# harveybc/gym-fx

Measured on AMD Instinct MI355X. Metric: env-steps/sec (whole node) PPO EURUSD-1m 4096 vec-envs, higher is better.
Workload: dtype bf16; 1 GPU; model=PPO MLP(256,256) actor-critic bf16 MFMA, global_batch=524288, seq_len=32, parallelism=dp1, n_envs_per_gpu=4096, rollout_steps=128, obs_dim=260, preprocessor=feature_window_preprocessor, reward=pnl_reward, pairs=1

## Files before the change

### gymfx_amd/algo/ppo.py

```python
from __future__ import annotations

import time
from dataclasses import dataclass
from typing import Any, Dict, List

import torch

from ..envs.vec_env import VecFxEnv
from ..models.lstm import ActorCriticLSTM
from ..models.mlp import ActorCriticMLP
from ..ops import api


@dataclass
class PPOConfig:
    rollout_steps: int = 128
    ppo_epochs: int = 4
    minibatches: int = 8
    gamma: float = 0.99
    gae_lambda: float = 0.95
    clip_eps: float = 0.2
    ent_coef: float = 0.01
    vf_coef: float = 0.5
    lr: float = 3e-4
    max_grad_norm: float = 0.5
    seed: int = 0
    hidden: int = 256
    normalize_adv: bool = True
    shuffle_rows: bool = True
    use_graphs: bool = True
    policy: str = "mlp"
    bptt_len: int = 16
    fused_rollout: bool = False
    rollout_streams: int = 1
    fuse_sample: bool = True
    fuse_head: bool = False
    overlap_gather: bool = False
    fused_opt_tail: bool = True

    @classmethod
    def from_config(cls, cfg: Dict[str, Any]) -> "PPOConfig":
        out = cls()
        mapping = {
            "rollout_steps": "rollout_steps",
            "ppo_epochs": "ppo_epochs",
            "minibatches": "minibatches",
            "gamma": "gamma",
            "gae_lambda": "gae_lambda",
            "clip_eps": "clip_eps",
            "ent_coef": "ent_coef",
            "vf_coef": "vf_coef",
            "lr": "learning_rate",
            "max_grad_norm": "max_grad_norm",
            "hidden": "hidden_size",
            "normalize_adv": "normalize_adv",
            "shuffle_rows": "shuffle_rows",
            "use_graphs": "use_graphs",
            "policy": "policy_model",
            "bptt_len": "bptt_len",
            "rollout_streams": "rollout_streams",
            "fused_rollout": "fused_rollout",
            "fuse_sample": "fuse_sample",
            "fuse_head": "fuse_head",
            "overlap_gather": "overlap_gather",
            "fused_opt_tail": "fused_opt_tail",
        }
        from ..config.merger import convert_type

        for attr, key in mapping.items():
            if cfg.get(key) is not None:
                cur = getattr(out, attr)
                val = convert_type(cfg[key]) if isinstance(cur, bool) else cfg[key]
                setattr(out, attr, type(cur)(val))
        if cfg.get("seed") is not None:
            out.seed = int(cfg["seed"])
        return out


class PPOTrainer:
    def __init__(self, env: VecFxEnv, cfg: PPOConfig, *, rank: int = 0,
# ... 114 lines not shown
        import os as _os
        self._fuse_gather = (
            not self.recurrent and self.device.type == "cuda"
            and cfg.shuffle_rows and not self._overlap
            and _os.environ.get("GYMFX_FUSE_GATHER", "0") == "1")
        self._fm = {"seed": self.shuffle_seed, "minibatches": cfg.minibatches,
                    "ctr_off": -1, "step_base": self.step_base,
                    "mb_ctr": self.mb_ctr}

        self._fused_tail = bool(cfg.fused_opt_tail) and (
            not self.recurrent
            or _os.environ.get("GYMFX_LSTM_OPT_TAIL", "0") == "1")
        self.model.fused_tail = self._fused_tail
        self.model.fuse_norm = (self._fused_tail and world_size <= 1
                                and cfg.max_grad_norm > 0)
        self._mb_ticket = (
            torch.zeros((), dtype=torch.int32, device=dev)
            if self._fused_tail
            and _os.environ.get("GYMFX_GATHER_TICKET", "0") == "1" else None)

        self.global_step = 0
        self.update_count = 0
        self.use_graphs = bool(cfg.use_graphs) and self.device.type == "cuda"
        self._split = (self.device.type == "cuda" and cfg.rollout_streams > 1
                       and N % 2 == 0)
        self._fused = (self.device.type == "cuda" and cfg.fused_rollout
                       and not self.recurrent and cfg.hidden == 256)
        self._fuse_sample = (self.device.type == "cuda" and cfg.fuse_sample
                             and getattr(env, "_native", None) is not None
                             and env.params.action_space_mode != "continuous")
# ... 137 lines not shown
    def _fwd_bwd_body(self, slot: int = 0) -> None:
        cfg, model = self.cfg, self.model
        if self.recurrent:
            head = model.bptt_forward(self.obs_mb_seq, self.done_mb,
                                      self.h0_mb, self.c0_mb, self.bptt)
            api.ppo_loss_bwd(
                head, self.act_mb.view(-1), self.logp_mb.view(-1),
                self.adv_mb.view(-1), self.ret_mb.view(-1), self.dhead,
                clip_eps=cfg.clip_eps, ent_coef=cfg.ent_coef,
                vf_coef=cfg.vf_coef, inv_count=1.0 / self.mb_rows,
                losses=self.losses,
            )
            model.bptt_backward(self.obs_mb_seq, self.done_mb, self.dhead,
                                self.bptt)
            return
        if self._fuse_gather:
            head = model.forward(self.obs_flat, self.acts_train,
                                 a_feistel=self._fm)
        else:
            head = model.forward(self.obs_mb_s[slot], self.acts_train)
        api.ppo_loss_bwd(
            head, self.act_mb_s[slot], self.logp_mb_s[slot],
            self.adv_mb_s[slot], self.ret_mb_s[slot],
            self.dhead, clip_eps=cfg.clip_eps, ent_coef=cfg.ent_coef,
            vf_coef=cfg.vf_coef, inv_count=1.0 / self.mb_rows,
            losses=self.losses,
        )
        if self._fuse_gather:
            model.backward(self.obs_flat, self.acts_train, self.dhead,
                           self.scratch, a_feistel=self._fm)
        else:
            model.backward(self.obs_mb_s[slot], self.acts_train, self.dhead,
                           self.scratch)

    def _mb_body(self, slot: int = 0) -> None:
        self._gather_body(slot)
        self._fwd_bwd_body(slot)

    def _mb_body_noshuffle(self, epoch_mb: int) -> None:
        cfg, model = self.cfg, self.model
        M = self.mb_rows
        mb = epoch_mb % cfg.minibatches
        sl = slice(mb * M, (mb + 1) * M)
        self.obs_mb.copy_(self.obs_flat[sl])
        self.act_mb.copy_(self.act_flat[sl])
        self.logp_mb.copy_(self.logp_flat[sl])
        self.adv_mb.copy_(self.adv_flat[sl])
        self.ret_mb.copy_(self.ret_flat[sl])
        head = model.forward(self.obs_mb, self.acts_train)
        api.ppo_loss_bwd(
            head, self.act_mb, self.logp_mb, self.adv_mb, self.ret_mb,
            self.dhead, clip_eps=cfg.clip_eps, ent_coef=cfg.ent_coef,
            vf_coef=cfg.vf_coef, inv_count=1.0 / M, losses=self.losses,
        )
        model.backward(self.obs_mb, self.acts_train, self.dhead, self.scratch)

    def _opt_body(self) -> None:
        self.model.adam(self.cfg.lr, max_grad_norm=self.cfg.max_grad_norm)

    def _snapshot(self) -> Dict[str, Any]:
        m = self.model
        snap = {
            "params": m.params.clone(), "m": m.m.clone(), "v": m.v.clone(),
# ... 63 lines not shown

    def collect_rollout(self) -> None:
        if self.use_graphs and self._graphs_ready:
            self.g_rollout.replay()
        else:
            self._rollout_body()
            self._gae_body()
        self.global_step += self.T

    def compute_advantages(self) -> None:
        pass

    def update(self, with_stats: bool = True) -> Dict[str, float]:
        cfg = self.cfg
        self.losses.zero_()
        self.mb_ctr.zero_()
        graphs = self.use_graphs and self._graphs_ready
        n_mb = cfg.ppo_epochs * cfg.minibatches
        if not cfg.shuffle_rows:
            for i in range(n_mb):
                self._mb_body_noshuffle(i)
                self._allreduce_grads()
                self._opt_body()
            self.update_count += 1
            return self._stats(n_mb) if with_stats else {}
        def gather(slot: int) -> None:
            if graphs:
                self.g_gather[slot].replay()
            else:
                self._gather_body(slot)

        def fwd_bwd(slot: int) -> None:
            if graphs:
                self.g_fwd_bwd[slot].replay()
            else:
                self._fwd_bwd_body(slot)

        def opt() -> None:
            if graphs:
                self.g_opt.replay()
            else:
                self._opt_body()

        if not self._overlap:
            gather(0)
            for i in range(n_mb):
                fwd_bwd(0)
                self._reducer.start(self.model.grads)
                if i + 1 < n_mb:
                    gather(0)
                self._reducer.finish()
                opt()
            self.update_count += 1
            return self._stats(n_mb) if with_stats else {}
        s2 = self._gs
        main = torch.cuda.current_stream()
        ev_fork = torch.cuda.Event()
        ev_g = [torch.cuda.Event(), torch.cuda.Event()]
        gather(0)
        for i in range(n_mb):
            slot = i & 1
            nxt = slot ^ 1
            if i + 1 < n_mb:
                ev_fork.record()
                with torch.cuda.stream(s2):
                    s2.wait_event(ev_fork)
                    gather(nxt)
                    ev_g[nxt].record()
            fwd_bwd(slot)
            self._reducer.start(self.model.grads)
            self._reducer.finish()
            opt()
            if i + 1 < n_mb:
                main.wait_event(ev_g[nxt])
        self.update_count += 1
        return self._stats(n_mb) if with_stats else {}

    def _stats(self, n_mb: int) -> Dict[str, float]:
        lv = (self.losses / n_mb).cpu()
        return {
            "pi_loss": float(lv[0]),
            "v_loss": float(lv[1]),
            "entropy": float(lv[2]),
            "approx_kl": float(lv[3]),
            "clipfrac": float(lv[4]),
        }

    def _allreduce_grads(self) -> None:
        if self.world_size <= 1:
# ... 94 lines not shown
```

### gymfx_amd/config/defaults.py

```python
from __future__ import annotations

DEFAULT_VALUES = {
    "mode": "inference",
    "driver_mode": "buy_hold",
    "steps": 500,

    "data_feed_plugin": "default_data_feed",
    "broker_plugin": "default_broker",
    "strategy_plugin": "default_strategy",
    "preprocessor_plugin": "default_preprocessor",
    "reward_plugin": "pnl_reward",
    "metrics_plugin": "default_metrics",

    "input_data_file": "examples/data/eurusd.csv",
    "date_column": "DATE_TIME",
    "price_column": "CLOSE",
    "instrument": "EUR_USD",
    "timeframe": "M1",
    "headers": True,
    "max_rows": None,

    "window_size": 32,
    "initial_cash": 10000.0,
    "position_size": 1.0,
# ... 35 lines not shown
    "ppo_epochs": 4,
    "minibatches": 8,
    "bptt_len": 16,
    "learning_rate": 3e-4,
    "gamma": 0.99,
    "gae_lambda": 0.95,
    "clip_eps": 0.2,
    "ent_coef": 0.01,
    "vf_coef": 0.5,
    "max_grad_norm": 0.5,
    "train_updates": 10,
    "use_graphs": True,
    "fuse_sample": True,
    "overlap_gather": False,
    "fused_opt_tail": True,
    "checkpoint_file": None,
    "checkpoint_interval": 0,
    "resume": False,
    "trace_file": None,

    "serve_host": "127.0.0.1",
    "serve_port": 8400,

    "optimization_trials": 16,
    "optimization_steps": 256,
    "optimization_refine_trials": 0,
}
```

### gymfx_amd/models/mlp.py

```python
from __future__ import annotations

import math
from dataclasses import dataclass
from typing import Dict, Optional, Tuple

import torch

from ..ops import api


@dataclass
class _ParamSlice:
    name: str
    shape: Tuple[int, ...]
    sl: slice
    is_weight: bool


class ActorCriticMLP:
    def __init__(
        self,
        obs_dim: int,
        n_actions: int = 3,
        hidden: int = 256,
# ... 125 lines not shown

    def forward(self, obs_bf16: torch.Tensor, acts: Dict[str, torch.Tensor],
                a_feistel: "Optional[dict]" = None) -> torch.Tensor:
        api.gemm(obs_bf16, self.wt("W1"), self.f32("b1"), acts["h1"], act=2,
                 trans_b=True, a_perm=a_feistel)
        api.gemm(acts["h1"], self.wt("W2"), self.f32("b2"), acts["h2"], act=2, trans_b=True)
        api.gemm(acts["h2"], self.wt("W3"), self.f32("b3"), acts["head"], act=0, trans_b=True)
        return acts["head"]

    def forward_hidden(self, obs_bf16: torch.Tensor,
                       acts: Dict[str, torch.Tensor]) -> torch.Tensor:
        api.gemm(obs_bf16, self.wt("W1"), self.f32("b1"), acts["h1"], act=2, trans_b=True)
        api.gemm(acts["h1"], self.wt("W2"), self.f32("b2"), acts["h2"], act=2, trans_b=True)
        return acts["h2"]

    def backward(
        self,
        obs_bf16: torch.Tensor,
        acts: Dict[str, torch.Tensor],
        dhead: torch.Tensor,
        scratch: Dict[str, torch.Tensor],
        a_feistel: "Optional[dict]" = None,
    ) -> None:
        M = dhead.shape[0]
        dh2 = scratch["dh2"]
        dh1 = scratch["dh1"]
        red = not self.fused_tail
        dw_p, db_p, slabs = self._wg_workspace("W3", self.hidden, self.head_dim, True)
        api.wgrad(acts["h2"], dhead, self.grad("W3"), self.grad("b3"),
                  workspace=(dw_p, db_p), slabs=slabs, reduce=red)
        api.gemm(dhead, self.w("W3"), None, dh2, Yact=acts["h2"], trans_b=True,
                 act=1, dact_tanh=True)
        dw_p, db_p, slabs = self._wg_workspace("W2", self.hidden, self.hidden, True)
        api.wgrad(acts["h1"], dh2, self.grad("W2"), self.grad("b2"),
                  workspace=(dw_p, db_p), slabs=slabs, reduce=red)
        api.gemm(dh2, self.w("W2"), None, dh1, Yact=acts["h1"], trans_b=True,
                 act=1, dact_tanh=True)
        dw_p, db_p, slabs = self._wg_workspace("W1", self.obs_dim, self.hidden, True)
        api.wgrad(obs_bf16, dh1, self.grad("W1"), self.grad("b1"),
                  workspace=(dw_p, db_p), slabs=slabs, x_perm=a_feistel,
                  reduce=red)
        if self.fused_tail:
            api.grads_finalize(self._finalize_segments(), self.grads,
                               self._clip_part if self.fuse_norm else None)

    def alloc_scratch(self, M: int) -> Dict[str, torch.Tensor]:
        dev = self.device
# ... 49 lines not shown
```

### gymfx_amd/ops/api.py

```python
from __future__ import annotations

from typing import Optional, Sequence, Tuple

import os

import torch

from . import native

_LSTM_FUSED = os.environ.get("GYMFX_LSTM_FUSED", "1") != "0"
_LSTM_BWD_FUSED = os.environ.get("GYMFX_LSTM_BWD_FUSED", "0") == "1"


def _use_native(t: torch.Tensor) -> bool:
    if t.is_cuda:
        native.require()
        return True
    return False



def gemm(
    A: torch.Tensor,
    B: torch.Tensor,
# ... 452 lines not shown
    dlogits = g_lp.unsqueeze(1) * (onehot - pi)
    dlogits = dlogits + ent_coef * pi * (logpi + H.unsqueeze(1))
    v = head[:, A]
    dv = vf_coef * (v - ret)
    d = torch.cat([dlogits, dv.unsqueeze(1)], dim=1) * inv_count
    dhead.copy_(d.to(torch.bfloat16))
    if losses is not None:
        losses[0] += float((-torch.minimum(surr1, surr2)).sum()) * inv_count
        losses[1] += float((0.5 * (v - ret) ** 2).sum()) * inv_count
        losses[2] += float(H.sum()) * inv_count
        losses[3] += float((old_logp - lp).sum()) * inv_count
        clipped = (ratio > 1 + clip_eps) | (ratio < 1 - clip_eps)
        losses[4] += float(clipped.to(torch.float32).sum()) * inv_count


def adv_normalize(adv: torch.Tensor, part: torch.Tensor) -> None:
    if _use_native(adv):
        native.require().adv_normalize(adv, part)
        return
    mean = adv.mean()
    var = (adv * adv).mean() - mean * mean
    adv.sub_(mean).div_(var.clamp(min=0).sqrt() + 1e-8)


def f32_to_bf16(src: torch.Tensor, dst: torch.Tensor) -> None:
    if _use_native(src):
        native.require().f32_to_bf16(src, dst)
        return
    dst.view(-1).copy_(src.reshape(-1).to(torch.bfloat16))

# ... 169 lines not shown
```

### gymfx_amd/ops/csrc/bindings.cpp

```cpp
#include <torch/extension.h>

#include <c10/hip/HIPStream.h>
#include <hip/hip_runtime.h>

#include <unordered_map>
#include <string>
#include <vector>

#include "env_common.h"

namespace gymfx {

void launch_env_step(const EnvPtrs& P, const EnvParamsK& K, int env_lo,
                     int env_cnt, hipStream_t stream);
void launch_build_obs(const EnvPtrs& P, const EnvParamsK& K, int env_lo,
                      int env_cnt, hipStream_t stream);
void launch_env_step_obs(const EnvPtrs& P, const EnvParamsK& K, int env_lo,
                         int env_cnt, hipStream_t stream);
void launch_gemm(const void* A, const void* B, const float* bias, void* C,
                 const void* Yact, int M, int N, int K, bool trans_b, int act,
                 bool dact_tanh, bool add_bias, bool accum, hipStream_t stream,
                 const FeistelMap* fmp = nullptr);
void launch_lstm_cell_fwd(const void* gates_pre, const void* gates_h,
                          const float* c_prev, float* c_new, void* h_new,
// ... 80 lines not shown
                               int row_offset, int greedy, hipStream_t stream);
void launch_increment_i32(int* ctr, int delta, hipStream_t stream);
void launch_mb_gather(const void* obs_src, const int64_t* act_src,
                      const float* logp_src, const float* adv_src,
                      const float* ret_src, void* obs_mb, int64_t* act_mb,
                      float* logp_mb, float* adv_mb, float* ret_mb, int M,
                      int D, uint32_t n, int half, uint64_t seed,
                      int minibatches, const unsigned long long* step_base,
                      unsigned long long* mb_ctr, hipStream_t stream,
                      int skip_obs = 0, unsigned int* ticket = nullptr);
void launch_ppo_loss_bwd(const float* head, const int64_t* actions,
                         const float* old_logp, const float* adv,
                         const float* ret, void* dhead, int M, int n_actions,
                         float clip_eps, float ent_coef, float vf_coef,
                         float inv_count, float* losses, hipStream_t stream);
void launch_adv_normalize(float* adv, int64_t n, float* part, int nparts,
                          hipStream_t stream);
void launch_f32_to_bf16(const float* in, void* out, int64_t n,
                        hipStream_t stream);
void launch_transpose_bf16(const void* src, void* dst, int K, int N,
                           hipStream_t stream);

namespace {

using TensorMap = std::unordered_map<std::string, torch::Tensor>;

template <typename T>
T* ptr(TensorMap& m, const char* key, bool required = true) {
  auto it = m.find(key);
  if (it == m.end() || !it->second.defined()) {
// ... 961 lines not shown
                     torch::Tensor ret, torch::Tensor dhead, double clip_eps,
                     double ent_coef, double vf_coef, double inv_count,
                     c10::optional<torch::Tensor> losses) {
  check_f32(head, "head");
  check_bf16(dhead, "dhead");
  const int M = (int)head.size(0);
  const int n_actions = (int)head.size(1) - 1;
  gymfx::launch_ppo_loss_bwd(
      head.data_ptr<float>(), actions.data_ptr<int64_t>(),
      old_logp.data_ptr<float>(), adv.data_ptr<float>(), ret.data_ptr<float>(),
      dhead.data_ptr(), M, n_actions, (float)clip_eps, (float)ent_coef,
      (float)vf_coef, (float)inv_count,
      losses.has_value() ? losses->data_ptr<float>() : nullptr, cur_stream());
}

void adv_normalize_op(torch::Tensor adv, torch::Tensor part) {
  check_f32(adv, "adv");
  check_f32(part, "part");
  gymfx::launch_adv_normalize(adv.data_ptr<float>(), adv.numel(),
                              part.data_ptr<float>(), (int)(part.numel() / 2),
                              cur_stream());
}

void f32_to_bf16_op(torch::Tensor in, torch::Tensor out) {
  check_f32(in, "in");
  check_bf16(out, "out");
  gymfx::launch_f32_to_bf16(in.data_ptr<float>(), out.data_ptr(), in.numel(),
                            cur_stream());
}

// ... 90 lines not shown
        py::arg("W1t"), py::arg("b1"), py::arg("W2t"), py::arg("b2"),
        py::arg("W3t"), py::arg("b3"), py::arg("actions"), py::arg("logp"),
        py::arg("value"), py::arg("seed"), py::arg("step"),
        py::arg("step_base") = py::none(), py::arg("row_offset") = 0,
        py::arg("greedy") = false);
  m.def("mb_gather", &mb_gather_op, py::arg("obs_src"), py::arg("act_src"),
        py::arg("logp_src"), py::arg("adv_src"), py::arg("ret_src"),
        py::arg("obs_mb"), py::arg("act_mb"), py::arg("logp_mb"),
        py::arg("adv_mb"), py::arg("ret_mb"), py::arg("seed"),
        py::arg("minibatches"), py::arg("step_base"), py::arg("mb_ctr"),
        py::arg("skip_obs") = false, py::arg("ticket") = py::none());
  m.def("ppo_loss_bwd", &ppo_loss_bwd_op, py::arg("head"), py::arg("actions"),
        py::arg("old_logp"), py::arg("adv"), py::arg("ret"), py::arg("dhead"),
        py::arg("clip_eps"), py::arg("ent_coef"), py::arg("vf_coef"),
        py::arg("inv_count"), py::arg("losses") = py::none());
  m.def("adv_normalize", &adv_normalize_op);
  m.def("f32_to_bf16", &f32_to_bf16_op);
  m.def("transpose_bf16", &transpose_bf16_op);
  py::class_<gymfx::GymFxEngine>(m, "GymFxEngine")
      .def(py::init<const py::dict&, const py::dict&, const py::dict&, const py::dict&>())
      .def("step", &gymfx::GymFxEngine::step, py::arg("actions"),
           py::arg("obs_out"), py::arg("reward_out") = py::none(),
           py::arg("terminated_out") = py::none(),
           py::arg("obs_bf16_out") = py::none(), py::arg("env_lo") = 0,
           py::arg("env_hi") = 0, py::arg("head") = py::none(),
           py::arg("logp_out") = py::none(), py::arg("value_out") = py::none(),
           py::arg("step_base") = py::none(), py::arg("sample_seed") = 0,
           py::arg("sample_step") = 0, py::arg("fuse_obs") = false,
           py::arg("h2") = py::none(), py::arg("w3t") = py::none(),
           py::arg("b3") = py::none(), py::arg("rnn_h") = py::none(),
// ... 8 lines not shown
```

### gymfx_amd/ops/csrc/ppo_kernels.hip

```cpp
#include "env_common.h"

#include <hip/hip_bf16.h>

#include <algorithm>

namespace gymfx {

typedef __attribute__((ext_vector_type(8))) __bf16 bf16x8;
typedef __attribute__((ext_vector_type(4))) float f32x4;

GFX_DEV float bf2f(__bf16 v) { return (float)v; }
GFX_DEV __bf16 f2bf(float v) { return (__bf16)v; }

GFX_DEV float fast_tanh(float x) {
  x = fminf(fmaxf(x, -15.f), 15.f);
  const float e = __builtin_amdgcn_exp2f(x * 2.885390081777927f);
  return 1.f - 2.f * __builtin_amdgcn_rcpf(e + 1.f);
}

GFX_DEV uint32_t feistel_encrypt_once(uint32_t x, int half, uint32_t mask,
                                      uint64_t key) {
  uint32_t a = x & mask;
  uint32_t b = x >> half;
  for (int r = 0; r < 4; ++r) {
// ... 883 lines not shown
    a = sample_categorical(row, n_actions, logz, seed, step, mg);
  }
  actions[m] = a;
  logp[m] = row[a] - logz;
  if (value) value[m] = row[n_actions];
  if (entropy) {
    float h = 0.f;
    for (int j = 0; j < n_actions; ++j) {
      const float lp = row[j] - logz;
      h -= fast_exp(lp) * lp;
    }
    entropy[m] = h;
  }
}

__global__ void ppo_loss_bwd_kernel(
    const float* __restrict__ head, const int64_t* __restrict__ actions,
    const float* __restrict__ old_logp, const float* __restrict__ adv,
    const float* __restrict__ ret, __bf16* __restrict__ dhead, int M,
    int n_actions, float clip_eps, float ent_coef, float vf_coef,
    float inv_count, float* __restrict__ losses) {
  const int m = blockIdx.x * blockDim.x + threadIdx.x;
  float l_pi = 0.f, l_v = 0.f, l_ent = 0.f, l_kl = 0.f, l_clip = 0.f;
  if (m < M) {
    const float* row = head + (int64_t)m * (n_actions + 1);
    __bf16* drow = dhead + (int64_t)m * (n_actions + 1);
    float mx = row[0];
    for (int j = 1; j < n_actions; ++j) mx = fmaxf(mx, row[j]);
    float z = 0.f;
    for (int j = 0; j < n_actions; ++j) z += expf(row[j] - mx);
    const float logz = logf(z) + mx;
    const int a = (int)actions[m];
    const float lp = row[a] - logz;
    const float ratio = expf(lp - old_logp[m]);
    const float A = adv[m];
    const bool clipped = (ratio > 1.f + clip_eps) || (ratio < 1.f - clip_eps);
    const float surr1 = ratio * A;
    const float rclip = fminf(fmaxf(ratio, 1.f - clip_eps), 1.f + clip_eps);
    const float surr2 = rclip * A;
    const float g_lp = (surr1 <= surr2) ? (-A * ratio) : 0.f;
    float H = 0.f;
    for (int j = 0; j < n_actions; ++j) {
      const float lpj = row[j] - logz;
      H -= expf(lpj) * lpj;
    }
    for (int j = 0; j < n_actions; ++j) {
      const float pj = expf(row[j] - logz);
      const float onehot = (j == a) ? 1.f : 0.f;
      float d = g_lp * (onehot - pj);
      d += ent_coef * pj * ((row[j] - logz) + H);
      drow[j] = f2bf(d * inv_count);
    }
    const float v = row[n_actions];
    const float dv = vf_coef * (v - ret[m]);
    drow[n_actions] = f2bf(dv * inv_count);

    l_pi = -fminf(surr1, surr2);
    l_v = 0.5f * (v - ret[m]) * (v - ret[m]);
    l_ent = H;
    l_kl = old_logp[m] - lp;
    l_clip = clipped ? 1.f : 0.f;
  }
  __shared__ float red[256];
  float vals[5] = {l_pi, l_v, l_ent, l_kl, l_clip};
  for (int s = 0; s < 5; ++s) {
    red[threadIdx.x] = vals[s];
    __syncthreads();
    for (int w = 128; w > 0; w >>= 1) {
      if (threadIdx.x < w) red[threadIdx.x] += red[threadIdx.x + w];
      __syncthreads();
    }
    if (threadIdx.x == 0 && losses) atomicAdd(&losses[s], red[0] * inv_count);
    __syncthreads();
  }
}

__global__ void adv_norm_stats_kernel(const float* __restrict__ adv, int64_t n,
                                      float* __restrict__ part ) {
  __shared__ float red[512];
  float s = 0.f, ss = 0.f;
  for (int64_t i = (int64_t)blockIdx.x * blockDim.x + threadIdx.x; i < n;
       i += (int64_t)gridDim.x * blockDim.x) {
    s += adv[i];
    ss += adv[i] * adv[i];
  }
  red[threadIdx.x] = s;
  red[256 + threadIdx.x] = ss;
  __syncthreads();
// ... 1015 lines not shown
    if (act == 0) { if (add_bias) GEMM_LAUNCH(false, 0, false, true); else GEMM_LAUNCH(false, 0, false, false); }
    else if (act == 1) { if (add_bias) GEMM_LAUNCH(false, 1, false, true); else GEMM_LAUNCH(false, 1, false, false); }
    else { if (add_bias) GEMM_LAUNCH(false, 2, false, true); else GEMM_LAUNCH(false, 2, false, false); }
  } else if (trans_b && !dact_tanh) {
    if (act == 0) { if (add_bias) GEMM_LAUNCH(true, 0, false, true); else GEMM_LAUNCH(true, 0, false, false); }
    else if (act == 1) { if (add_bias) GEMM_LAUNCH(true, 1, false, true); else GEMM_LAUNCH(true, 1, false, false); }
    else { if (add_bias) GEMM_LAUNCH(true, 2, false, true); else GEMM_LAUNCH(true, 2, false, false); }
  } else if (trans_b && dact_tanh) {
    GEMM_LAUNCH(true, 1, true, false);
  } else {
    GEMM_LAUNCH(false, 1, true, false);
  }
#undef GEMM_LAUNCH
}

void launch_wgrad(const void* X, const void* dY, float* dW_part, float* db_part,
                  float* dW, float* db, int M, int N, int K, int slabs,
                  hipStream_t stream, const FeistelMap* fmp = nullptr,
                  bool reduce = true) {
  const __bf16* x = reinterpret_cast<const __bf16*>(X);
  const __bf16* dy = reinterpret_cast<const __bf16*>(dY);
  static const int big_env = [] {
    const char* e = getenv("GYMFX_WGRAD_BIG");
    return e ? atoi(e) : -1;
  }();
  const bool big = K >= 128 && N >= 128 &&
                   (big_env >= 0
                        ? big_env != 0
                        : (int64_t)ceil_div(K, 128) * ceil_div(N, 128) * slabs >=
                              384);
// ... 41 lines not shown
    else                                                                      \
      hipLaunchKernelGGL((wgrad_partial_kernel<WDB, FK, FN>), grid,           \
                         dim3(256), 0, stream, x, dy, dW_part, db_part, M, N, \
                         K, slabs, 0);                                        \
  } while (0)
    if (db_part) {
      if (big) WG_PART(true, 4, 4);
      else WG_PART(true, 2, 2);
    } else {
      if (big) WG_PART(false, 4, 4);
      else WG_PART(false, 2, 2);
    }
#undef WG_PART
  }
  if (!reduce) return;
  int64_t elems = (int64_t)K * N;
  if (elems <= 4096) {
    hipLaunchKernelGGL(slab_reduce_small_kernel, dim3((int)elems), dim3(256),
                       0, stream, dW_part, dW, elems, slabs);
  } else {
    int blocks = (int)std::min<int64_t>((elems + 1023) / 1024, 1024);
    hipLaunchKernelGGL(slab_reduce_kernel, dim3(blocks), dim3(256), 0, stream,
                       dW_part, dW, elems, slabs);
  }
  if (db_part && db)
    hipLaunchKernelGGL(slab_reduce_small_kernel, dim3(N), dim3(256), 0, stream,
                       db_part, db, (int64_t)N, slabs);
}

void launch_gae(const float* rewards, const float* values, const bool* dones,
// ... 69 lines not shown
                     stream, head, M, n_actions, seed, step, actions, logp,
                     value, entropy, greedy, step_base, row_offset);
}

void launch_ppo_loss_bwd(const float* head, const int64_t* actions,
                         const float* old_logp, const float* adv,
                         const float* ret, void* dhead, int M, int n_actions,
                         float clip_eps, float ent_coef, float vf_coef,
                         float inv_count, float* losses, hipStream_t stream) {
  hipLaunchKernelGGL(ppo_loss_bwd_kernel, dim3(ceil_div(M, 256)), dim3(256), 0,
                     stream, head, actions, old_logp, adv, ret,
                     reinterpret_cast<__bf16*>(dhead), M, n_actions, clip_eps,
                     ent_coef, vf_coef, inv_count, losses);
}

void launch_adv_normalize(float* adv, int64_t n, float* part, int nparts,
                          hipStream_t stream) {
  hipLaunchKernelGGL(adv_norm_stats_kernel, dim3(nparts), dim3(256), 0, stream,
                     adv, n, part);
  int blocks = (int)std::min<int64_t>((n + 255) / 256, 2048);
  hipLaunchKernelGGL(adv_norm_apply_kernel, dim3(blocks), dim3(256), 0, stream,
                     adv, n, part, nparts);
}

void launch_transpose_bf16(const void* src, void* dst, int K, int N,
                           hipStream_t stream) {
  dim3 grid(ceil_div(K, 64), ceil_div(N, 64));
  hipLaunchKernelGGL(transpose_bf16_kernel, grid, dim3(256), 0, stream,
                     reinterpret_cast<const __bf16*>(src),
                     reinterpret_cast<__bf16*>(dst), K, N);
// ... 11 lines not shown
```

Before: 29.17 million env-steps/sec.

## Fuse PPO head GEMM, loss, weight-grad and tanh data-grad into one kernel

Adds a head_loss_bwd HIP kernel that, per row slab, loads h2 into LDS and then does the rest in one launch: the head GEMM, the PPO loss and its gradient, partial W3/b3 gradients and the tanh-masked dh2 via MFMA. The MLP training path now calls forward_hidden plus this fused op, and the rest of backward skips its head part. Loss accumulation is sharded across 64 rows to cut atomic contention, and the shards are folded once per update. The fused path only runs when ceil(M/slabs) <= 128. Otherwise it falls back to the original unfused sequence, so at large minibatch sizes it may never run.

```diff
diff --git a/gymfx_amd/algo/ppo.py b/gymfx_amd/algo/ppo.py
--- a/gymfx_amd/algo/ppo.py
+++ b/gymfx_amd/algo/ppo.py
@@ -37,6 +37,7 @@
     fuse_head: bool = False
     overlap_gather: bool = False
     fused_opt_tail: bool = True
+    fused_head_bwd: bool = True
 
     @classmethod
     def from_config(cls, cfg: Dict[str, Any]) -> "PPOConfig":
@@ -64,6 +65,7 @@
             "fuse_head": "fuse_head",
             "overlap_gather": "overlap_gather",
             "fused_opt_tail": "fused_opt_tail",
+            "fused_head_bwd": "fused_head_bwd",
         }
         from ..config.merger import convert_type
 
@@ -208,6 +210,10 @@
         self.model.fused_tail = self._fused_tail
         self.model.fuse_norm = (self._fused_tail and world_size <= 1
                                 and cfg.max_grad_norm > 0)
+        self._fused_head = bool(cfg.fused_head_bwd) and not self.recurrent
+        self._loss_shards = (
+            torch.zeros(64, 32, dtype=torch.float32, device=dev)
+            if self._fused_head and self.device.type == "cuda" else None)
         self._mb_ticket = (
             torch.zeros((), dtype=torch.int32, device=dev)
             if self._fused_tail
@@ -375,6 +381,18 @@
             model.bptt_backward(self.obs_mb_seq, self.done_mb, self.dhead,
                                 self.bptt)
             return
+        if self._fused_head and not self._fuse_gather:
+            model.forward_hidden(self.obs_mb_s[slot], self.acts_train)
+            model.head_loss_backward(
+                self.acts_train, self.act_mb_s[slot], self.logp_mb_s[slot],
+                self.adv_mb_s[slot], self.ret_mb_s[slot], self.dhead,
+                self.scratch, clip_eps=cfg.clip_eps, ent_coef=cfg.ent_coef,
+                vf_coef=cfg.vf_coef, inv_count=1.0 / self.mb_rows,
+                losses=self._loss_acc(),
+            )
+            model.backward(self.obs_mb_s[slot], self.acts_train, self.dhead,
+                           self.scratch, skip_head=True)
+            return
         if self._fuse_gather:
             head = model.forward(self.obs_flat, self.acts_train,
                                  a_feistel=self._fm)
@@ -394,6 +412,13 @@
             model.backward(self.obs_mb_s[slot], self.acts_train, self.dhead,
                            self.scratch)
 
+    def _loss_acc(self) -> torch.Tensor:
+        return self.losses if self._loss_shards is None else self._loss_shards
+
+    def _fold_losses(self) -> None:
+        if self._loss_shards is not None:
+            self.losses.add_(self._loss_shards[:, :5].sum(dim=0))
+
     def _mb_body(self, slot: int = 0) -> None:
         self._gather_body(slot)
         self._fwd_bwd_body(slot)
@@ -408,6 +433,17 @@
         self.logp_mb.copy_(self.logp_flat[sl])
         self.adv_mb.copy_(self.adv_flat[sl])
         self.ret_mb.copy_(self.ret_flat[sl])
+        if self._fused_head:
+            model.forward_hidden(self.obs_mb, self.acts_train)
+            model.head_loss_backward(
+                self.acts_train, self.act_mb, self.logp_mb, self.adv_mb,
+                self.ret_mb, self.dhead, self.scratch, clip_eps=cfg.clip_eps,
+                ent_coef=cfg.ent_coef, vf_coef=cfg.vf_coef, inv_count=1.0 / M,
+                losses=self._loss_acc(),
+            )
+            model.backward(self.obs_mb, self.acts_train, self.dhead,
+                           self.scratch, skip_head=True)
+            return
         head = model.forward(self.obs_mb, self.acts_train)
         api.ppo_loss_bwd(
             head, self.act_mb, self.logp_mb, self.adv_mb, self.ret_mb,
@@ -501,6 +537,8 @@
     def update(self, with_stats: bool = True) -> Dict[str, float]:
         cfg = self.cfg
         self.losses.zero_()
+        if self._loss_shards is not None:
+            self._loss_shards.zero_()
         self.mb_ctr.zero_()
         graphs = self.use_graphs and self._graphs_ready
         n_mb = cfg.ppo_epochs * cfg.minibatches
@@ -509,6 +547,7 @@
                 self._mb_body_noshuffle(i)
                 self._allreduce_grads()
                 self._opt_body()
+            self._fold_losses()
             self.update_count += 1
             return self._stats(n_mb) if with_stats else {}
         def gather(slot: int) -> None:
@@ -538,6 +577,7 @@
                     gather(0)
                 self._reducer.finish()
                 opt()
+            self._fold_losses()
             self.update_count += 1
             return self._stats(n_mb) if with_stats else {}
         s2 = self._gs
@@ -560,6 +600,7 @@
             opt()
             if i + 1 < n_mb:
                 main.wait_event(ev_g[nxt])
+        self._fold_losses()
         self.update_count += 1
         return self._stats(n_mb) if with_stats else {}
 
diff --git a/gymfx_amd/config/defaults.py b/gymfx_amd/config/defaults.py
--- a/gymfx_amd/config/defaults.py
+++ b/gymfx_amd/config/defaults.py
@@ -73,6 +73,7 @@
     "fuse_sample": True,
     "overlap_gather": False,
     "fused_opt_tail": True,
+    "fused_head_bwd": True,
     "checkpoint_file": None,
     "checkpoint_interval": 0,
     "resume": False,
diff --git a/gymfx_amd/models/mlp.py b/gymfx_amd/models/mlp.py
--- a/gymfx_amd/models/mlp.py
+++ b/gymfx_amd/models/mlp.py
@@ -163,6 +163,31 @@
         api.gemm(acts["h1"], self.wt("W2"), self.f32("b2"), acts["h2"], act=2, trans_b=True)
         return acts["h2"]
 
+    def head_loss_backward(
+        self,
+        acts: Dict[str, torch.Tensor],
+        actions: torch.Tensor,
+        old_logp: torch.Tensor,
+        adv: torch.Tensor,
+        ret: torch.Tensor,
+        dhead: torch.Tensor,
+        scratch: Dict[str, torch.Tensor],
+        *,
+        clip_eps: float,
+        ent_coef: float,
+        vf_coef: float,
+        inv_count: float,
+        losses: Optional[torch.Tensor] = None,
+    ) -> None:
+        dw_p, db_p, slabs = self._wg_workspace("W3", self.hidden, self.head_dim, True)
+        api.head_loss_bwd(
+            acts["h2"], self.wt("W3"), self.w("W3"), self.f32("b3"), actions,
+            old_logp, adv, ret, acts["head"], dhead, scratch["dh2"],
+            self.grad("W3"), self.grad("b3"), workspace=(dw_p, db_p),
+            slabs=slabs, reduce=not self.fused_tail, clip_eps=clip_eps,
+            ent_coef=ent_coef, vf_coef=vf_coef, inv_count=inv_count,
+            losses=losses)
+
     def backward(
         self,
         obs_bf16: torch.Tensor,
@@ -170,16 +195,18 @@
         dhead: torch.Tensor,
         scratch: Dict[str, torch.Tensor],
         a_feistel: "Optional[dict]" = None,
+        skip_head: bool = False,
     ) -> None:
         M = dhead.shape[0]
         dh2 = scratch["dh2"]
         dh1 = scratch["dh1"]
         red = not self.fused_tail
-        dw_p, db_p, slabs = self._wg_workspace("W3", self.hidden, self.head_dim, True)
-        api.wgrad(acts["h2"], dhead, self.grad("W3"), self.grad("b3"),
-                  workspace=(dw_p, db_p), slabs=slabs, reduce=red)
-        api.gemm(dhead, self.w("W3"), None, dh2, Yact=acts["h2"], trans_b=True,
-                 act=1, dact_tanh=True)
+        if not skip_head:
+            dw_p, db_p, slabs = self._wg_workspace("W3", self.hidden, self.head_dim, True)
+            api.wgrad(acts["h2"], dhead, self.grad("W3"), self.grad("b3"),
+                      workspace=(dw_p, db_p), slabs=slabs, reduce=red)
+            api.gemm(dhead, self.w("W3"), None, dh2, Yact=acts["h2"], trans_b=True,
+                     act=1, dact_tanh=True)
         dw_p, db_p, slabs = self._wg_workspace("W2", self.hidden, self.hidden, True)
         api.wgrad(acts["h1"], dh2, self.grad("W2"), self.grad("b2"),
                   workspace=(dw_p, db_p), slabs=slabs, reduce=red)
diff --git a/gymfx_amd/ops/api.py b/gymfx_amd/ops/api.py
--- a/gymfx_amd/ops/api.py
+++ b/gymfx_amd/ops/api.py
@@ -490,6 +490,61 @@
         losses[4] += float(clipped.to(torch.float32).sum()) * inv_count
 
 
+def head_loss_bwd_fusable(M: int, hidden: int, head_dim: int,
+                          slabs: int) -> bool:
+    return (hidden == 256 and 2 <= head_dim <= 16 and slabs >= 1
+            and (M + slabs - 1) // slabs <= 128)
+
+
+def head_loss_bwd(
+    h2: torch.Tensor,
+    W3t: torch.Tensor,
+    W3: torch.Tensor,
+    b3: torch.Tensor,
+    actions: torch.Tensor,
+    old_logp: torch.Tensor,
+    adv: torch.Tensor,
+    ret: torch.Tensor,
+    head: torch.Tensor,
+    dhead: torch.Tensor,
+    dh2: torch.Tensor,
+    dW: torch.Tensor,
+    db: torch.Tensor,
+    *,
+    workspace: Optional[Tuple[torch.Tensor, torch.Tensor]] = None,
+    slabs: int = 64,
+    reduce: bool = True,
+    clip_eps: float,
+    ent_coef: float,
+    vf_coef: float,
+    inv_count: float,
+    losses: Optional[torch.Tensor] = None,
+) -> None:
+    M, hidden = h2.shape
+    head_dim = W3.shape[1]
+    if _use_native(h2) and head_loss_bwd_fusable(M, hidden, head_dim, slabs):
+        if workspace is None:
+            workspace = (
+                torch.empty(slabs, hidden, head_dim, dtype=torch.float32,
+                            device=h2.device),
+                torch.empty(slabs, head_dim, dtype=torch.float32,
+                            device=h2.device),
+            )
+        native.require().head_loss_bwd(
+            h2, W3t, W3, b3, actions, old_logp, adv, ret, head, dhead, dh2,
+            workspace[0], workspace[1], dW, db, slabs, reduce, clip_eps,
+            ent_coef, vf_coef, inv_count, losses)
+        return
+    if losses is not None and losses.dim() == 2:
+        losses = losses[0]
+    gemm(h2, W3t, b3, head, act=0, trans_b=True)
+    ppo_loss_bwd(head, actions, old_logp, adv, ret, dhead, clip_eps=clip_eps,
+                 ent_coef=ent_coef, vf_coef=vf_coef, inv_count=inv_count,
+                 losses=losses)
+    wgrad(h2, dhead, dW, db, workspace=workspace, slabs=slabs, reduce=reduce)
+    gemm(dhead, W3, None, dh2, Yact=h2, trans_b=True, act=1, dact_tanh=True)
+
+
 def adv_normalize(adv: torch.Tensor, part: torch.Tensor) -> None:
     if _use_native(adv):
         native.require().adv_normalize(adv, part)
diff --git a/gymfx_amd/ops/csrc/bindings.cpp b/gymfx_amd/ops/csrc/bindings.cpp
--- a/gymfx_amd/ops/csrc/bindings.cpp
+++ b/gymfx_amd/ops/csrc/bindings.cpp
@@ -118,6 +118,16 @@
                          const float* ret, void* dhead, int M, int n_actions,
                          float clip_eps, float ent_coef, float vf_coef,
                          float inv_count, float* losses, hipStream_t stream);
+void launch_head_loss_bwd(const void* h2, const void* W3t, const void* W3,
+                          const float* b3, const int64_t* actions,
+                          const float* old_logp, const float* adv,
+                          const float* ret, float* head, void* dhead,
+                          void* dh2, float* dW_part, float* db_part, int M,
+                          int head_dim, int slabs, float clip_eps,
+                          float ent_coef, float vf_coef, float inv_count,
+                          float* losses, int loss_shards, hipStream_t stream);
+void launch_slab_reduce(const float* dW_part, const float* db_part, float* dW,
+                        float* db, int N, int K, int slabs, hipStream_t stream);
 void launch_adv_normalize(float* adv, int64_t n, float* part, int nparts,
                           hipStream_t stream);
 void launch_f32_to_bf16(const float* in, void* out, int64_t n,
@@ -1109,6 +1119,79 @@
       losses.has_value() ? losses->data_ptr<float>() : nullptr, cur_stream());
 }
 
+void head_loss_bwd_op(torch::Tensor h2, torch::Tensor W3t, torch::Tensor W3,
+                      torch::Tensor b3, torch::Tensor actions,
+                      torch::Tensor old_logp, torch::Tensor adv,
+                      torch::Tensor ret, torch::Tensor head,
+                      torch::Tensor dhead, torch::Tensor dh2,
+                      torch::Tensor dW_part, torch::Tensor db_part,
+                      torch::Tensor dW, torch::Tensor db, int64_t slabs,
+                      bool reduce, double clip_eps, double ent_coef,
+                      double vf_coef, double inv_count,
+                      c10::optional<torch::Tensor> losses) {
+  check_bf16(h2, "h2");
+  check_bf16(W3t, "W3t");
+  check_bf16(W3, "W3");
+  check_f32(b3, "b3");
+  check_f32(head, "head");
+  check_bf16(dhead, "dhead");
+  check_bf16(dh2, "dh2");
+  check_f32(dW_part, "dW_part");
+  check_f32(db_part, "db_part");
+  check_f32(dW, "dW");
+  check_f32(db, "db");
+  check_f32(old_logp, "old_logp");
+  check_f32(adv, "adv");
+  check_f32(ret, "ret");
+  const int64_t M = h2.size(0), H = h2.size(1), hd = W3.size(1);
+  TORCH_CHECK(H == 256 && hd >= 2 && hd <= 16,
+              "head_loss_bwd: needs hidden == 256 and head_dim <= 16");
+  TORCH_CHECK(slabs >= 1 && (M + slabs - 1) / slabs <= 128,
+              "head_loss_bwd: needs ceil(M/slabs) <= 128");
+  TORCH_CHECK(W3.size(0) == H && W3t.size(0) == hd && W3t.size(1) == H &&
+                  b3.numel() == hd, "head_loss_bwd: weight shapes");
+  TORCH_CHECK(head.size(0) == M && head.size(1) == hd && dhead.size(0) == M &&
+                  dhead.size(1) == hd && dh2.size(0) == M && dh2.size(1) == H,
+              "head_loss_bwd: activation shapes");
+  TORCH_CHECK(actions.scalar_type() == torch::kInt64 && actions.numel() == M &&
+                  old_logp.numel() == M && adv.numel() == M &&
+                  ret.numel() == M, "head_loss_bwd: per-row inputs");
+  TORCH_CHECK(h2.is_contiguous() && W3.is_contiguous() &&
+                  W3t.is_contiguous() && head.is_contiguous() &&
+                  dhead.is_contiguous() && dh2.is_contiguous() &&
+                  actions.is_contiguous() && old_logp.is_contiguous() &&
+                  adv.is_contiguous() && ret.is_contiguous(),
+              "head_loss_bwd: contiguous tensors only");
+  TORCH_CHECK(dW_part.numel() >= slabs * H * hd, "dW_part too small");
+  TORCH_CHECK(db_part.numel() >= slabs * hd, "db_part too small");
+  TORCH_CHECK(dW.numel() == H * hd && db.numel() == hd, "dW/db shape");
+  int loss_shards = 1;
+  if (losses.has_value()) {
+    check_f32(*losses, "losses");
+    if (losses->dim() == 2) {
+      TORCH_CHECK(losses->size(1) == 32 && losses->size(0) >= 1,
+                  "sharded losses must be [S, 32]");
+      loss_shards = (int)losses->size(0);
+    } else {
+      TORCH_CHECK(losses->numel() >= 5, "losses numel");
+    }
+  }
+  gymfx::launch_head_loss_bwd(
+      h2.data_ptr(), W3t.data_ptr(), W3.data_ptr(), b3.data_ptr<float>(),
+      actions.data_ptr<int64_t>(), old_logp.data_ptr<float>(),
+      adv.data_ptr<float>(), ret.data_ptr<float>(), head.data_ptr<float>(),
+      dhead.data_ptr(), dh2.data_ptr(), dW_part.data_ptr<float>(),
+      db_part.data_ptr<float>(), (int)M, (int)hd, (int)slabs, (float)clip_eps,
+      (float)ent_coef, (float)vf_coef, (float)inv_count,
+      losses.has_value() ? losses->data_ptr<float>() : nullptr, loss_shards,
+      cur_stream());
+  if (reduce)
+    gymfx::launch_slab_reduce(dW_part.data_ptr<float>(),
+                              db_part.data_ptr<float>(), dW.data_ptr<float>(),
+                              db.data_ptr<float>(), (int)hd, (int)H,
+                              (int)slabs, cur_stream());
+}
+
 void adv_normalize_op(torch::Tensor adv, torch::Tensor part) {
   check_f32(adv, "adv");
   check_f32(part, "part");
@@ -1229,6 +1312,13 @@
         py::arg("old_logp"), py::arg("adv"), py::arg("ret"), py::arg("dhead"),
         py::arg("clip_eps"), py::arg("ent_coef"), py::arg("vf_coef"),
         py::arg("inv_count"), py::arg("losses") = py::none());
+  m.def("head_loss_bwd", &head_loss_bwd_op, py::arg("h2"), py::arg("W3t"),
+        py::arg("W3"), py::arg("b3"), py::arg("actions"), py::arg("old_logp"),
+        py::arg("adv"), py::arg("ret"), py::arg("head"), py::arg("dhead"),
+        py::arg("dh2"), py::arg("dW_part"), py::arg("db_part"), py::arg("dW"),
+        py::arg("db"), py::arg("slabs"), py::arg("reduce"),
+        py::arg("clip_eps"), py::arg("ent_coef"), py::arg("vf_coef"),
+        py::arg("inv_count"), py::arg("losses") = py::none());
   m.def("adv_normalize", &adv_normalize_op);
   m.def("f32_to_bf16", &f32_to_bf16_op);
   m.def("transpose_bf16", &transpose_bf16_op);
diff --git a/gymfx_amd/ops/csrc/ppo_kernels.hip b/gymfx_amd/ops/csrc/ppo_kernels.hip
--- a/gymfx_amd/ops/csrc/ppo_kernels.hip
+++ b/gymfx_amd/ops/csrc/ppo_kernels.hip
@@ -7,6 +7,7 @@
 namespace gymfx {
 
 typedef __attribute__((ext_vector_type(8))) __bf16 bf16x8;
+typedef __attribute__((ext_vector_type(4))) __bf16 bf16x4;
 typedef __attribute__((ext_vector_type(4))) float f32x4;
 
 GFX_DEV float bf2f(__bf16 v) { return (float)v; }
@@ -921,6 +922,46 @@
   }
 }
 
+GFX_DEV void ppo_loss_row(const float* row, __bf16* drow, int a, float olp,
+                          float A, float rt, int n_actions, float clip_eps,
+                          float ent_coef, float vf_coef, float inv_count,
+                          float& l_pi, float& l_v, float& l_ent, float& l_kl,
+                          float& l_clip) {
+  float mx = row[0];
+  for (int j = 1; j < n_actions; ++j) mx = fmaxf(mx, row[j]);
+  float z = 0.f;
+  for (int j = 0; j < n_actions; ++j) z += expf(row[j] - mx);
+  const float logz = logf(z) + mx;
+  const float lp = row[a] - logz;
+  const float ratio = expf(lp - olp);
+  const bool clipped = (ratio > 1.f + clip_eps) || (ratio < 1.f - clip_eps);
+  const float surr1 = ratio * A;
+  const float rclip = fminf(fmaxf(ratio, 1.f - clip_eps), 1.f + clip_eps);
+  const float surr2 = rclip * A;
+  const float g_lp = (surr1 <= surr2) ? (-A * ratio) : 0.f;
+  float H = 0.f;
+  for (int j = 0; j < n_actions; ++j) {
+    const float lpj = row[j] - logz;
+    H -= expf(lpj) * lpj;
+  }
+  for (int j = 0; j < n_actions; ++j) {
+    const float pj = expf(row[j] - logz);
+    const float onehot = (j == a) ? 1.f : 0.f;
+    float d = g_lp * (onehot - pj);
+    d += ent_coef * pj * ((row[j] - logz) + H);
+    drow[j] = f2bf(d * inv_count);
+  }
+  const float v = row[n_actions];
+  const float dv = vf_coef * (v - rt);
+  drow[n_actions] = f2bf(dv * inv_count);
+
+  l_pi = -fminf(surr1, surr2);
+  l_v = 0.5f * (v - rt) * (v - rt);
+  l_ent = H;
+  l_kl = olp - lp;
+  l_clip = clipped ? 1.f : 0.f;
+}
+
 __global__ void ppo_loss_bwd_kernel(
     const float* __restrict__ head, const int64_t* __restrict__ actions,
     const float* __restrict__ old_logp, const float* __restrict__ adv,
@@ -929,45 +970,11 @@
     float inv_count, float* __restrict__ losses) {
   const int m = blockIdx.x * blockDim.x + threadIdx.x;
   float l_pi = 0.f, l_v = 0.f, l_ent = 0.f, l_kl = 0.f, l_clip = 0.f;
-  if (m < M) {
-    const float* row = head + (int64_t)m * (n_actions + 1);
-    __bf16* drow = dhead + (int64_t)m * (n_actions + 1);
-    float mx = row[0];
-    for (int j = 1; j < n_actions; ++j) mx = fmaxf(mx, row[j]);
-    float z = 0.f;
-    for (int j = 0; j < n_actions; ++j) z += expf(row[j] - mx);
-    const float logz = logf(z) + mx;
-    const int a = (int)actions[m];
-    const float lp = row[a] - logz;
-    const float ratio = expf(lp - old_logp[m]);
-    const float A = adv[m];
-    const bool clipped = (ratio > 1.f + clip_eps) || (ratio < 1.f - clip_eps);
-    const float surr1 = ratio * A;
-    const float rclip = fminf(fmaxf(ratio, 1.f - clip_eps), 1.f + clip_eps);
-    const float surr2 = rclip * A;
-    const float g_lp = (surr1 <= surr2) ? (-A * ratio) : 0.f;
-    float H = 0.f;
-    for (int j = 0; j < n_actions; ++j) {
-      const float lpj = row[j] - logz;
-      H -= expf(lpj) * lpj;
-    }
-    for (int j = 0; j < n_actions; ++j) {
-      const float pj = expf(row[j] - logz);
-      const float onehot = (j == a) ? 1.f : 0.f;
-      float d = g_lp * (onehot - pj);
-      d += ent_coef * pj * ((row[j] - logz) + H);
-      drow[j] = f2bf(d * inv_count);
-    }
-    const float v = row[n_actions];
-    const float dv = vf_coef * (v - ret[m]);
-    drow[n_actions] = f2bf(dv * inv_count);
-
-    l_pi = -fminf(surr1, surr2);
-    l_v = 0.5f * (v - ret[m]) * (v - ret[m]);
-    l_ent = H;
-    l_kl = old_logp[m] - lp;
-    l_clip = clipped ? 1.f : 0.f;
-  }
+  if (m < M)
+    ppo_loss_row(head + (int64_t)m * (n_actions + 1),
+                 dhead + (int64_t)m * (n_actions + 1), (int)actions[m],
+                 old_logp[m], adv[m], ret[m], n_actions, clip_eps, ent_coef,
+                 vf_coef, inv_count, l_pi, l_v, l_ent, l_kl, l_clip);
   __shared__ float red[256];
   float vals[5] = {l_pi, l_v, l_ent, l_kl, l_clip};
   for (int s = 0; s < 5; ++s) {
@@ -979,6 +986,228 @@
     }
     if (threadIdx.x == 0 && losses) atomicAdd(&losses[s], red[0] * inv_count);
     __syncthreads();
+  }
+}
+
+constexpr int kHlbRows = 128;
+constexpr int kHlbHid = 256;
+constexpr int kHlbHead = 16;
+constexpr int kHlbHdLd = kHlbHead + 1;
+constexpr int kLossShardLd = 32;
+
+GFX_DEV int hlb_off(int r, int col) {
+  const int c = col >> 3;
+  return r * kHlbHid + (((c & 16) | ((c ^ r) & 15)) << 3) + (col & 7);
+}
+
+__global__ __launch_bounds__(256, 2) void head_loss_bwd_kernel(
+    const __bf16* __restrict__ h2, const __bf16* __restrict__ W3t,
+    const __bf16* __restrict__ W3, const float* __restrict__ b3,
+    const int64_t* __restrict__ actions, const float* __restrict__ old_logp,
+    const float* __restrict__ adv, const float* __restrict__ ret,
+    float* __restrict__ head, __bf16* __restrict__ dhead,
+    __bf16* __restrict__ dh2, float* __restrict__ dW_part,
+    float* __restrict__ db_part, int M, int head_dim, int slabs,
+    float clip_eps, float ent_coef, float vf_coef, float inv_count,
+    float* __restrict__ losses, int loss_shards) {
+  constexpr int kTileBytes = kHlbRows * kHlbHid * 2;
+  constexpr int kHdBytes = kHlbRows * kHlbHdLd * 4;
+  constexpr int kDsBytes = kHlbRows * kHlbHead * 2;
+  __shared__ __align__(16) unsigned char smem[kTileBytes + kHdBytes + kDsBytes];
+  __bf16* Hs = reinterpret_cast<__bf16*>(smem);
+  float* Hd = reinterpret_cast<float*>(smem + kTileBytes);
+  __bf16* Ds = reinterpret_cast<__bf16*>(smem + kTileBytes + kHdBytes);
+
+  const int tid = threadIdx.x;
+  const int wave = tid >> 6, lane = tid & 63;
+  const int row_a = lane & 15;
+  const int kseg = lane >> 4;
+  const int crow_base = (lane >> 4) * 4;
+  const int ccol = lane & 15;
+
+  const int slab = blockIdx.x;
+  const int m_per_slab = (M + slabs - 1) / slabs;
+  const int m_begin = slab * m_per_slab;
+  const int m_end = min(M, m_begin + m_per_slab);
+  const int nrows = max(0, m_end - m_begin);
+  const int rpad = min(kHlbRows, (nrows + 31) & ~31);
+  const int n_actions = head_dim - 1;
+
+  bf16x8 bh[kHlbHid / 32];
+#pragma unroll
+  for (int ks = 0; ks < kHlbHid / 32; ++ks) {
+    bh[ks] = bf16x8{};
+    if (row_a < head_dim)
+      bh[ks] = *reinterpret_cast<const bf16x8*>(
+          &W3t[row_a * kHlbHid + ks * 32 + kseg * 8]);
+  }
+  *reinterpret_cast<bf16x8*>(&Ds[tid * 8]) = bf16x8{};
+  if (nrows == kHlbRows) {
+    for (int j = 0; j < 16; ++j) {
+      const int e0 = (wave * 16 + j) * 512;
+      const int e = e0 + lane * 8;
+      const int r = e >> 8;
+      const int p = (e >> 3) & 31;
+      const int c = (p & 16) | ((p ^ r) & 15);
+      __builtin_amdgcn_global_load_lds(
+          (const __attribute__((address_space(1))) void*)(uintptr_t)(
+              &h2[(int64_t)(m_begin + r) * kHlbHid + c * 8]),
+          (__attribute__((address_space(3))) void*)(uintptr_t)(Hs + e0), 16, 0,
+          0);
+    }
+  } else {
+    for (int idx = tid; idx < rpad * 32; idx += 256) {
+      const int r = idx >> 5;
+      const int p = idx & 31;
+      const int c = (p & 16) | ((p ^ r) & 15);
+      bf16x8 v = bf16x8{};
+      if (r < nrows)
+        v = *reinterpret_cast<const bf16x8*>(
+            &h2[(int64_t)(m_begin + r) * kHlbHid + c * 8]);
+      *reinterpret_cast<bf16x8*>(&Hs[idx * 8]) = v;
+    }
+  }
+  __syncthreads();
+
+  if (wave * 32 < rpad) {
+    for (int mi = 0; mi < 2; ++mi) {
+      const int r0 = wave * 32 + mi * 16;
+      f32x4 acc = {};
+#pragma unroll
+      for (int ks = 0; ks < kHlbHid / 32; ++ks) {
+        const bf16x8 af = *reinterpret_cast<const bf16x8*>(
+            &Hs[hlb_off(r0 + row_a, ks * 32 + kseg * 8)]);
+        acc = __builtin_amdgcn_mfma_f32_16x16x32_bf16(af, bh[ks], acc, 0, 0, 0);
+      }
+      if (ccol < head_dim) {
+#pragma unroll
+        for (int r = 0; r < 4; ++r) {
+          float v = acc[r];
+          v += b3[ccol];
+          Hd[(r0 + crow_base + r) * kHlbHdLd + ccol] = v;
+        }
+      }
+    }
+  }
+  __syncthreads();
+
+  {
+    float l_pi = 0.f, l_v = 0.f, l_ent = 0.f, l_kl = 0.f, l_clip = 0.f;
+    if (tid < nrows) {
+      const int m = m_begin + tid;
+      ppo_loss_row(Hd + tid * kHlbHdLd, Ds + tid * kHlbHead, (int)actions[m],
+                   old_logp[m], adv[m], ret[m], n_actions, clip_eps, ent_coef,
+                   vf_coef, inv_count, l_pi, l_v, l_ent, l_kl, l_clip);
+    }
+    if (losses && wave * 64 < nrows) {
+      losses += (slab % loss_shards) * kLossShardLd;
+      float vals[5] = {l_pi, l_v, l_ent, l_kl, l_clip};
+#pragma unroll
+      for (int s = 0; s < 5; ++s) {
+        float x = vals[s];
+        for (int o = 32; o > 0; o >>= 1) x += __shfl_down(x, o, 64);
+        if (lane == 0) atomicAdd(&losses[s], x * inv_count);
+      }
+    }
+  }
+  __syncthreads();
+
+  for (int idx = tid; idx < nrows * head_dim; idx += 256) {
+    const int r = idx / head_dim;
+    const int j = idx - r * head_dim;
+    head[(int64_t)m_begin * head_dim + idx] = Hd[r * kHlbHdLd + j];
+    dhead[(int64_t)m_begin * head_dim + idx] = Ds[r * kHlbHead + j];
+  }
+
+  bf16x8 bw[4];
+#pragma unroll
+  for (int g = 0; g < 4; ++g) {
+    bw[g] = bf16x8{};
+    const int n = (wave * 4 + g) * 16 + row_a;
+#pragma unroll
+    for (int i = 0; i < 8; ++i) {
+      const int k = kseg * 8 + i;
+      const __bf16 w = W3[n * head_dim + min(k, head_dim - 1)];
+      bw[g][i] = (k < head_dim) ? w : (__bf16)0.f;
+    }
+  }
+
+  {
+    const int nchunks = (nrows + 31) / 32;
+    f32x4 acc[4] = {};
+    for (int ci = 0; ci < nchunks; ++ci) {
+      const int m0 = ci * 32 + kseg * 8;
+      bf16x8 bf_;
+#pragma unroll
+      for (int i = 0; i < 8; ++i) bf_[i] = Ds[(m0 + i) * kHlbHead + row_a];
+#pragma unroll
+      for (int f = 0; f < 4; ++f) {
+        bf16x8 af;
+#pragma unroll
+        for (int i = 0; i < 8; ++i)
+          af[i] = Hs[hlb_off(m0 + i, (wave * 4 + f) * 16 + row_a)];
+        acc[f] = __builtin_amdgcn_mfma_f32_16x16x32_bf16(af, bf_, acc[f], 0, 0,
+                                                         0);
+      }
+    }
+    float* out = dW_part + (int64_t)slab * kHlbHid * head_dim;
+    if (ccol < head_dim) {
+#pragma unroll
+      for (int f = 0; f < 4; ++f)
+#pragma unroll
+        for (int r = 0; r < 4; ++r) {
+          const int grow = (wave * 4 + f) * 16 + crow_base + r;
+          out[grow * head_dim + ccol] = acc[f][r];
+        }
+    }
+    if (tid < head_dim) {
+      float db_acc = 0.f;
+      for (int ci = 0; ci < nchunks; ++ci) {
+        float x[32];
+#pragma unroll
+        for (int i = 0; i < 32; ++i)
+          x[i] = bf2f(Ds[(ci * 32 + i) * kHlbHead + tid]);
+        float s = 0.f;
+#pragma unroll
+        for (int i = 0; i < 32; ++i) s += x[i];
+        db_acc += s;
+      }
+      db_part[(int64_t)slab * head_dim + tid] = db_acc;
+    }
+  }
+  __syncthreads();
+
+  for (int mi = 0; mi < rpad / 16; ++mi) {
+    bf16x8 df = bf16x8{};
+    if (kseg < kHlbHead / 8)
+      df = *reinterpret_cast<const bf16x8*>(
+          &Ds[(mi * 16 + row_a) * kHlbHead + kseg * 8]);
+#pragma unroll
+    for (int g = 0; g < 4; ++g) {
+      const f32x4 acc = __builtin_amdgcn_mfma_f32_16x16x32_bf16(
+          bw[g], df, f32x4{}, 0, 0, 0);
+      bf16x4* yp = reinterpret_cast<bf16x4*>(
+          &Hs[hlb_off(mi * 16 + ccol, (wave * 4 + g) * 16 + crow_base)]);
+      const bf16x4 yv = *yp;
+      bf16x4 ov;
+#pragma unroll
+      for (int r = 0; r < 4; ++r) {
+        float v = acc[r];
+        float y = bf2f(yv[r]);
+        v *= (1.f - y * y);
+        ov[r] = f2bf(v);
+      }
+      *yp = ov;
+    }
+  }
+  __syncthreads();
+
+  for (int idx = tid; idx < nrows * 32; idx += 256) {
+    const int r = idx >> 5;
+    const int p = idx & 31;
+    const int c = (p & 16) | ((p ^ r) & 15);
+    *reinterpret_cast<bf16x8*>(&dh2[(int64_t)(m_begin + r) * kHlbHid + c * 8]) =
+        *reinterpret_cast<const bf16x8*>(&Hs[idx * 8]);
   }
 }
 
@@ -2024,6 +2253,9 @@
 #undef GEMM_LAUNCH
 }
 
+void launch_slab_reduce(const float* dW_part, const float* db_part, float* dW,
+                        float* db, int N, int K, int slabs, hipStream_t stream);
+
 void launch_wgrad(const void* X, const void* dY, float* dW_part, float* db_part,
                   float* dW, float* db, int M, int N, int K, int slabs,
                   hipStream_t stream, const FeistelMap* fmp = nullptr,
@@ -2095,6 +2327,12 @@
 #undef WG_PART
   }
   if (!reduce) return;
+  launch_slab_reduce(dW_part, db_part, dW, db, N, K, slabs, stream);
+}
+
+void launch_slab_reduce(const float* dW_part, const float* db_part, float* dW,
+                        float* db, int N, int K, int slabs,
+                        hipStream_t stream) {
   int64_t elems = (int64_t)K * N;
   if (elems <= 4096) {
     hipLaunchKernelGGL(slab_reduce_small_kernel, dim3((int)elems), dim3(256),
@@ -2194,6 +2432,25 @@
                      ent_coef, vf_coef, inv_count, losses);
 }
 
+void launch_head_loss_bwd(const void* h2, const void* W3t, const void* W3,
+                          const float* b3, const int64_t* actions,
+                          const float* old_logp, const float* adv,
+                          const float* ret, float* head, void* dhead,
+                          void* dh2, float* dW_part, float* db_part, int M,
+                          int head_dim, int slabs, float clip_eps,
+                          float ent_coef, float vf_coef, float inv_count,
+                          float* losses, int loss_shards, hipStream_t stream) {
+  hipLaunchKernelGGL(head_loss_bwd_kernel, dim3(slabs), dim3(256), 0, stream,
+                     reinterpret_cast<const __bf16*>(h2),
+                     reinterpret_cast<const __bf16*>(W3t),
+                     reinterpret_cast<const __bf16*>(W3), b3, actions,
+                     old_logp, adv, ret, head,
+                     reinterpret_cast<__bf16*>(dhead),
+                     reinterpret_cast<__bf16*>(dh2), dW_part, db_part, M,
+                     head_dim, slabs, clip_eps, ent_coef, vf_coef, inv_count,
+                     losses, loss_shards);
+}
+
 void launch_adv_normalize(float* adv, int64_t n, float* part, int nparts,
                           hipStream_t stream) {
   hipLaunchKernelGGL(adv_norm_stats_kernel, dim3(nparts), dim3(256), 0, stream,
```

Measured after the change: 32.07 million env-steps/sec, median of 6. +9.9%, better.
